# rmcar17/SpectralClusterSupertree

Hardware: AMD Instinct MI355X
Metric: top-level PCG build + Fiedler solve wall-time (s) at N taxa, 1/2/4/8 MI355X (lower is better)
Workload: dtype f64 (loop operator: fp32 image of W; fp64 renewal + confirmation)

## Files before the change

spectralclustersupertree_amd/csrc/scs_build.hip:

```cpp

#include <algorithm>

#include "scs_internal.h"

typedef unsigned long long u64;
typedef unsigned int u32;

constexpr u32 DEPTH_INF = 0xFFFFFFFFu;


__device__ __forceinline__ void rmq_offsets(int m, int a, int b, int (&o)[2]) {
    const int k = 31 - __clz(b - a);
    o[0] = k * m + a;
    o[1] = k * m + b - (1 << k);
}

template <typename K>
__device__ __forceinline__ K rmq_min(const K *__restrict__ base, int m, int a, int b) {
    int o[2];
    rmq_offsets(m, a, b, o);
    const K x = base[o[0]], y = base[o[1]];
    return x < y ? x : y;
}

// ... 659 lines not shown
        }
        if (n <= 2048) max_batch_trees = 4096;
        const int arrived = tb->late_start.empty() ? M : tb->late_start[0];
        if (wide) {
            const int rest = M - (arrived < M ? arrived : 0);
            const int k = std::max(1, (rest + 511) / 512);
            max_batch_trees = std::max(96, (rest + k - 1) / k);
        }
        if (tree_par)
            max_batch_trees = (int)std::max<size_t>(16, std::min<size_t>((size_t)max_batch_trees,
                                                                         SCS_SCRATCH_KEEP / cells_per_tree));
        if (batch_trees_env > 0) max_batch_trees = batch_trees_env;
        if (tree_par)
            max_batch_trees = (int)std::max<size_t>(1, std::min<size_t>((size_t)max_batch_trees,
                                                                        SCS_SCRATCH_KEEP / std::max<size_t>(cells_per_tree, 1)));
        size_t used = 0;
        for (int t = 0; t < M; ++t) {
            const int64_t nt = tb->h_tree_off[t + 1] - tb->h_tree_off[t];
            const int64_t m = nt - 1;
            const size_t need =
                (size_t)table_entries(m) * entry_bytes + (size_t)npad * 4 + (size_t)n_blocks * rec_bytes;
            if ((used + need > ctx->ws_limit || t - batch_start.back() >= max_batch_trees ||
                 (t == arrived && batch_start.size() == 1)) &&
                t > batch_start.back()) {
                batch_start.push_back(t);
                used = 0;
            }
            used += need;
        }
        batch_start.push_back(M);
    }
    const int n_batches = (int)batch_start.size() - 1;

    struct ev_ref {
        hipEvent_t a, b;
    } ev_total, ev_prep, ev_acc;
    for (auto &e : ctx->build_events)
        if (!e) SCS_HIP_CHECK(hipEventCreate(&e));
    ev_total = {ctx->build_events[0], ctx->build_events[1]};
    ev_prep = {ctx->build_events[2], ctx->build_events[3]};
    ev_acc = {ctx->build_events[4], ctx->build_events[5]};
    float prep_ms = 0.f, acc_ms = 0.f;
    SCS_HIP_CHECK(hipEventRecord(ev_total.a, s));

    int spec_batches = 0, spec_trees = 0;
    float spec_ms = 0.f;
    bool single_batch_spec = false;
    pooled_buf d_pos(ctx, 1), d_st(ctx, 3), d_stoff(ctx, 4), d_rec(ctx, 5), d_cells(ctx, 6);
    dev_buf d_pcol(ctx), d_lists(ctx), d_list_cnt(ctx);
    int listed_batches = 0;
    for (int bi = 0; bi < n_batches; ++bi) {
        const int t0 = batch_start[bi], t1 = batch_start[bi + 1];
        const int nb = t1 - t0;
        std::vector<int64_t> st_off(nb + 1);
        int max_levels = 0;
        int64_t max_n = 0;
        st_off[0] = 0;
        for (int t = t0; t < t1; ++t) {
            const int64_t nt = tb->h_tree_off[t + 1] - tb->h_tree_off[t];
            st_off[t - t0 + 1] = st_off[t - t0] + table_entries(nt - 1);
            max_levels = std::max(max_levels, levels_for(nt - 1));
            max_n = std::max(max_n, nt);
        }
        const size_t need_pos = (size_t)nb * npad * 4;
        const size_t need_st = (size_t)st_off[nb] * entry_bytes + 64;
        const size_t need_stoff = (size_t)(nb + 1) * 8;
        const size_t need_rec = (size_t)n_blocks * nb * rec_bytes;
        const int wide_min_trees = wide_forced ? 1 : 96;
        const bool wide_b = wide && (nb >= wide_min_trees || (groups.size() >= 8 * 256 && nb >= 16));
        if (wide_b) {
            ++spec_batches;
            spec_trees += nb;
            single_batch_spec = true;
        }
        SCS_TRY(d_pos.alloc(need_pos));
        SCS_TRY(d_st.alloc(need_st));
        SCS_TRY(d_stoff.alloc(need_stoff));
        SCS_TRY(d_rec.alloc(need_rec));

        SCS_HIP_CHECK(hipEventRecord(ev_prep.a, s));
        SCS_TRY(scs_tables_wait(ctx, tb, t1, s));
        SCS_HIP_CHECK(hipMemcpyAsync(d_stoff.p, st_off.data(), need_stoff, hipMemcpyHostToDevice, s));
        SCS_HIP_CHECK(hipMemsetAsync(d_pos.p, 0xFF, need_pos, s));
        dim3 grid_l((unsigned)((max_n + 255) / 256), (unsigned)nb);
        if (monotone) {
            k_positions_values<<<grid_l, 256, 0, s>>>(tb->d_tree_off, tb->d_leaf_taxon,
                                                      tb->d_adj_depth, tb->d_adj_val, tb->d_tree_w,
                                                      t0, (int32_t *)d_pos.p, npad,
                                                      (const int64_t *)d_stoff.p, (double *)d_st.p);
            if (max_n <= SPARSE_FUSED_MAX_LEAVES && max_levels > 1)
                k_sparse_levels_fused<double><<<(unsigned)nb, 1024, 0, s>>>(
                    tb->d_tree_off, t0, (const int64_t *)d_stoff.p, (double *)d_st.p, pick_smaller_value{});
            else
            for (int k = 1; k < max_levels; ++k)
                k_sparse_level<double><<<grid_l, 256, 0, s>>>(tb->d_tree_off, t0, k,
                                                              (const int64_t *)d_stoff.p,
                                                              (double *)d_st.p);
            if (wide_b)
                k_block_records_wide<PIPE_NG><<<dim3((unsigned)n_blocks, (unsigned)nb), 64, 0, s>>>(
                    tb->d_tree_off, t0, nb, (const int32_t *)d_pos.p, npad, (const int64_t *)d_stoff.p,
                    (const double *)d_st.p, b_row_begin, b_row_end, (unsigned char *)d_rec.p);
            else if (!scatter)
            k_block_records_mono<<<dim3((unsigned)n_blocks, (unsigned)nb), 64, 0, s>>>(
                tb->d_tree_off, t0, nb, (const int32_t *)d_pos.p, npad, (const int64_t *)d_stoff.p,
                (const double *)d_st.p, b_row_begin, b_row_end, (unsigned char *)d_rec.p);
        } else {
            k_positions_pairs<<<grid_l, 256, 0, s>>>(tb->d_tree_off, tb->d_leaf_taxon,
                                                     tb->d_adj_depth, tb->d_adj_val, tb->d_tree_w,
                                                     t0, (int32_t *)d_pos.p, npad,
                                                     (const int64_t *)d_stoff.p, (gap_entry *)d_st.p);
            if (max_n <= SPARSE_FUSED_MAX_LEAVES && max_levels > 1)
                k_sparse_levels_fused<gap_entry><<<(unsigned)nb, 1024, 0, s>>>(
                    tb->d_tree_off, t0, (const int64_t *)d_stoff.p, (gap_entry *)d_st.p, pick_shallower_pair{});
            else
            for (int k = 1; k < max_levels; ++k)
                k_sparse_level_pairs<<<grid_l, 256, 0, s>>>(tb->d_tree_off, t0, k,
                                                            (const int64_t *)d_stoff.p,
                                                            (gap_entry *)d_st.p);
            k_block_records_gen<<<dim3((unsigned)n_blocks, (unsigned)nb), 64, 0, s>>>(
                tb->d_tree_off, t0, nb, (const int32_t *)d_pos.p, npad, (const int64_t *)d_stoff.p,
                (const gap_entry *)d_st.p, b_row_begin, b_row_end, (unsigned char *)d_rec.p);
        }
        SCS_HIP_CHECK(hipEventRecord(ev_prep.b, s));

        SCS_HIP_CHECK(hipEventRecord(ev_acc.a, s));
        const unsigned nt = (unsigned)tiles.size();
        if (scatter) {
            const int64_t nbk = (max_n + 63) / 64;
            k_scatter_atomic<<<dim3((unsigned)(nbk * (nbk + 1) / 2), (unsigned)nb), 256, 0, s>>>(
                tb->d_tree_off, tb->d_leaf_taxon, t0, (const int64_t *)d_stoff.p, (const double *)d_st.p,
                g->d_w, g->ld);
        } else if (monotone) {
            mono_params mp;
            mp.tiles = (const int2 *)d_tiles.p;
            mp.rec = (const unsigned char *)d_rec.p;
            mp.pos = (const int32_t *)d_pos.p;
            mp.npad = npad;
            mp.stv = (const double *)d_st.p;
            mp.n_batch = nb;
            mp.w = w_base;
            mp.ld = g->ld;
            mp.n = n;
            mp.row_begin = b_row_begin;
            mp.row_end = b_row_end;
            mp.load_w = bi > 0;
            mp.mirror = (sym && bi == n_batches - 1) ? 1 : 0;
            mp.tile_out = shared ? (double *)d_tile_out.p : nullptr;
            mp.stamps = nullptr;
            mp.split_tiles = 0;
            mp.lists = nullptr;
            mp.list_cnt = nullptr;
            const bool stamp = scs_dbg("SCS_ACC_STAMP") && atoi(scs_dbg("SCS_ACC_STAMP"));
            if (wide_b) {
                wide_params wp;
                wp.m = mp;
                wp.groups = (const int4 *)d_groups.p;
                wp.producer_prio = 2;
                const unsigned ng = (unsigned)groups.size();
// ... 78 lines not shown
        } else {
            gen_params gp;
            gp.tiles = (const int2 *)d_tiles.p;
            gp.rec = (const unsigned char *)d_rec.p;
            gp.pos = (const int32_t *)d_pos.p;
            gp.npad = npad;
            gp.ste = (const gap_entry *)d_st.p;
            gp.n_batch = nb;
            gp.w = w_base;
            gp.ld = g->ld;
            gp.n = n;
            gp.row_begin = b_row_begin;
            gp.row_end = b_row_end;
            gp.load_w = bi > 0;
            gp.mirror = (sym && bi == n_batches - 1) ? 1 : 0;
            gp.tile_out = shared ? (double *)d_tile_out.p : nullptr;
            gp.split_tiles = 0;
            if (nt && tree_par) {
                SCS_TRY(d_cells.alloc((size_t)nb * cells_per_tree));
                gen_params ap = gp;
                ap.split_tiles = (int)nt;
                ap.load_w = 0;
                ap.mirror = 0;
                ap.tile_out = (double *)d_cells.p;
                k_accumulate_gen<true><<<nt * (unsigned)nb, MONO_TCW, 0, s>>>(ap);
                k_sum_tree_tiles<true, gen_params><<<nt * SCS_TR, MONO_TCW, 0, s>>>(gp, (const double *)d_cells.p,
                                                                                   (int)nt);
            } else if (nt) {
                if (sym) k_accumulate_gen<true><<<nt, MONO_TCW, 0, s>>>(gp);
                else k_accumulate_gen<false><<<nt, MONO_TCW, 0, s>>>(gp);
            }
        }
        SCS_HIP_CHECK(hipGetLastError());
        SCS_HIP_CHECK(hipEventRecord(ev_acc.b, s));
        if (n_batches > 1) {
            SCS_HIP_CHECK(hipEventSynchronize(ev_acc.b));
            float ms = 0.f;
            SCS_HIP_CHECK(hipEventElapsedTime(&ms, ev_prep.a, ev_prep.b));
            prep_ms += ms;
            SCS_HIP_CHECK(hipEventElapsedTime(&ms, ev_acc.a, ev_acc.b));
            acc_ms += ms;
            if (wide_b) spec_ms += ms;
        }
    }
    float exch_ms = 0.f;
    double exch_bytes = 0.0;
    if (shared && exchange_allgather) {
        ev_pair ev_x;
        SCS_TRY(ev_x.init());
        SCS_HIP_CHECK(hipEventRecord(ev_x.a, s));
        SCS_TRY(scs_comm_allgather_f64(&ctx->comm, (const double *)d_tile_out.p,
                                       (double *)d_gathered.p, chunk_doubles, s));
        k_unpack_tiles<<<(unsigned)all_tiles.size(), cols_per_tile, 0, s>>>(
            (const double *)d_gathered.p, (const int2 *)d_all_tiles.p, world,
            (int64_t)chunk_doubles, n, row_begin, row_end, g->d_w, g->ld);
        SCS_HIP_CHECK(hipGetLastError());
        SCS_HIP_CHECK(hipEventRecord(ev_x.b, s));
        SCS_HIP_CHECK(hipEventSynchronize(ev_x.b));
        SCS_HIP_CHECK(hipEventElapsedTime(&exch_ms, ev_x.a, ev_x.b));
        exch_bytes = (double)chunk_doubles * 8.0 * (world - 1);
    } else if (shared) {
        std::vector<int32_t> splits;
        SCS_TRY(scs_gather_row_splits(ctx, row_begin, row_end, n, splits));
        auto needs = [&](int dst, const int2 &t) {
            const int64_t lo = splits[dst], hi = splits[dst + 1];
            const int64_t r_lo = (int64_t)t.x * SCS_TR, r_hi = std::min<int64_t>(r_lo + SCS_TR, n);
            const int64_t c_lo = (int64_t)t.y * cols_per_tile, c_hi = std::min<int64_t>(c_lo + cols_per_tile, n);
            return (r_lo < hi && lo < r_hi) || (c_lo < hi && lo < c_hi);
        };
        std::vector<int64_t> send_off(world + 1, 0), recv_off(world + 1, 0);
        std::vector<int32_t> send_slots;
        std::vector<int2> recv_tiles;
        for (int p = 0; p < world; ++p) {
            for (size_t i = rank; i < all_tiles.size(); i += world)
                if (needs(p, all_tiles[i])) send_slots.push_back((int32_t)(i / world));
            send_off[p + 1] = (int64_t)send_slots.size() * SCS_TR * cols_per_tile;
            for (size_t i = p; i < all_tiles.size(); i += world)
                if (needs(rank, all_tiles[i])) recv_tiles.push_back(all_tiles[i]);
            recv_off[p + 1] = (int64_t)recv_tiles.size() * SCS_TR * cols_per_tile;
        }
        cached_buf d_send(ctx), d_recv(ctx);
        dev_buf d_slots(ctx), d_rtiles(ctx);
        SCS_TRY(d_send.alloc((size_t)send_off[world] * 8));
        SCS_TRY(d_recv.alloc((size_t)recv_off[world] * 8));
        SCS_TRY(d_slots.alloc(send_slots.size() * 4));
        SCS_TRY(d_rtiles.alloc(recv_tiles.size() * sizeof(int2)));
        ev_pair ev_x;
        SCS_TRY(ev_x.init());
        SCS_HIP_CHECK(hipEventRecord(ev_x.a, s));
        SCS_HIP_CHECK(hipMemcpyAsync(d_slots.p, send_slots.data(), send_slots.size() * 4,
                                     hipMemcpyHostToDevice, s));
        SCS_HIP_CHECK(hipMemcpyAsync(d_rtiles.p, recv_tiles.data(), recv_tiles.size() * sizeof(int2),
                                     hipMemcpyHostToDevice, s));
        if (!send_slots.empty())
            k_pack_tiles<<<(unsigned)send_slots.size(), 256, 0, s>>>(
                (const double *)d_tile_out.p, (const int32_t *)d_slots.p, cols_per_tile, (double *)d_send.p);
        SCS_HIP_CHECK(hipGetLastError());
        SCS_TRY(scs_comm_alltoallv_f64(&ctx->comm, (const double *)d_send.p, send_off.data(),
                                       (double *)d_recv.p, recv_off.data(), s));
        if (!recv_tiles.empty())
            k_unpack_received<<<(unsigned)recv_tiles.size(), cols_per_tile, 0, s>>>(
                (const double *)d_recv.p, (const int2 *)d_rtiles.p, n, row_begin, row_end, g->d_w,
                g->ld);
        SCS_HIP_CHECK(hipGetLastError());
        SCS_HIP_CHECK(hipEventRecord(ev_x.b, s));
        SCS_HIP_CHECK(hipEventSynchronize(ev_x.b));
        SCS_HIP_CHECK(hipEventElapsedTime(&exch_ms, ev_x.a, ev_x.b));
        exch_bytes = (double)(recv_off[world] - (recv_off[rank + 1] - recv_off[rank])) * 8.0;
    }
    SCS_HIP_CHECK(hipEventRecord(ev_total.b, s));
    SCS_HIP_CHECK(hipEventSynchronize(ev_total.b));
    SCS_TRY(scs_tables_finish(ctx, tb));
    float total_ms = 0.f;
    SCS_HIP_CHECK(hipEventElapsedTime(&total_ms, ev_total.a, ev_total.b));
    if (n_batches == 1) {
        SCS_HIP_CHECK(hipEventElapsedTime(&prep_ms, ev_prep.a, ev_prep.b));
        SCS_HIP_CHECK(hipEventElapsedTime(&acc_ms, ev_acc.a, ev_acc.b));
        if (single_batch_spec) spec_ms = acc_ms;
    }

    if (stats) {
        memset(stats, 0, sizeof(*stats));
        stats->n_taxa = n;
        stats->n_trees = M;
        stats->row_begin = row_begin;
        stats->row_end = row_end;
        stats->symmetric = shared ? 2 : (sym ? 1 : 0);
        stats->exchange_ms = exch_ms;
        stats->exchange_bytes = exch_bytes;
        stats->n_tiles = (int32_t)tiles.size();
        stats->n_batches = n_batches;
        stats->spec_batches = spec_batches;
        stats->tree_parallel_batches = tree_par ? n_batches : 0;
        stats->spec_trees = spec_trees;
        stats->listed_batches = listed_batches;
        stats->spec_ms = spec_ms;
        stats->cell_trees = (double)tiles.size() * SCS_TR * cols_per_tile * (double)M;
        stats->prep_ms = prep_ms;
        stats->accumulate_ms = acc_ms;
        stats->total_ms = total_ms;
        stats->bytes_w = 8.0 * rows * (double)n;
        stats->bytes_tables = 16.0 * (double)tb->n_leaves + 8.0 * M;
    }
    gd.g = nullptr;
    *out = g;
    return SCS_OK;
}

extern "C" int scs_graph_contract(scs_ctx *ctx, scs_graph *g, const int32_t *group_start,
                                  int32_t n_groups, scs_graph **out) {
    SCS_REQUIRE(ctx && g && group_start && out, "scs_graph_contract: null argument");
// ... 217 lines not shown
```

spectralclustersupertree_amd/csrc/scs_ctx.hip:

```cpp

#include <dlfcn.h>

#include <atomic>
#include <condition_variable>
#include <mutex>

#include "scs_internal.h"
#include "scs_arena.h"

#include <chrono>
#include <pthread.h>

#include <algorithm>
#include <cmath>

static thread_local std::string g_last_error;

void scs_set_error(const char *fmt, ...) {
    char buf[1024];
    va_list ap;
    va_start(ap, fmt);
    vsnprintf(buf, sizeof(buf), fmt, ap);
    va_end(ap);
    g_last_error = buf;
// ... 473 lines not shown

namespace {
constexpr int ARENA_DEVICES = 16;
struct device_arena {
    std::mutex mu;
    scs_arena_core core;
    std::vector<hipEvent_t> event_pool;
    std::atomic<bool> live{false};
};
device_arena g_arena[ARENA_DEVICES];

bool arena_on() {
    static const bool on = [] {
        const char *e = scs_dbg("SCS_ARENA");
        return !(e && atoi(e) == 0);
    }();
    return on;
}

void arena_init(device_arena &a) {
    if (a.live.load()) return;
    a.core.back_alloc = [](size_t bytes) -> void * {
        void *p = nullptr;
        if (driver_malloc(&p, bytes) != hipSuccess) {
            (void)hipGetLastError();
            return nullptr;
        }
        return p;
    };
    a.core.back_free = [](void *p) { driver_free(p); };
    a.core.owner_mark = [&a](const void *owner) {
        std::vector<void *> events;
        const scs_ctx *ctx = (const scs_ctx *)owner;
        for (hipStream_t s : {ctx->stream, ctx->small_stream, ctx->copy_stream}) {
            if (!s) continue;
            if (hipStreamQuery(s) == hipSuccess) continue;
            (void)hipGetLastError();
            hipEvent_t ev = nullptr;
            if (!a.event_pool.empty()) {
                ev = a.event_pool.back();
                a.event_pool.pop_back();
            } else if (hipEventCreateWithFlags(&ev, hipEventDisableTiming) != hipSuccess) {
                (void)hipGetLastError();
                hipStreamSynchronize(s);
                continue;
            }
            hipEventRecord(ev, s);
            events.push_back((void *)ev);
        }
        return events;
    };
    a.core.event_done = [](void *e) {
        if (hipEventQuery((hipEvent_t)e) == hipSuccess) return true;
        (void)hipGetLastError();
        return false;
    };
    a.core.event_wait = [](void *e) { hipEventSynchronize((hipEvent_t)e); };
    a.core.event_recycle = [&a](void *e) { a.event_pool.push_back((hipEvent_t)e); };
    a.live.store(true);
}
}

hipError_t scs_dev_malloc_impl(scs_ctx *ctx, void **p, size_t bytes) {
    if (!ctx || !arena_on() || ctx->device < 0 || ctx->device >= ARENA_DEVICES) return driver_malloc(p, bytes);
    device_arena &a = g_arena[ctx->device];
    std::lock_guard<std::mutex> lock(a.mu);
    arena_init(a);
// ... 106 lines not shown
        if (b.p == p) b.in_use = false;
        if (!b.in_use) free_bytes += b.bytes;
    }
    while (free_bytes > SCS_PINNED_KEEP) {
        size_t pick = ctx->pinned.size();
        for (size_t i = 0; i < ctx->pinned.size(); ++i)
            if (!ctx->pinned[i].in_use && (pick == ctx->pinned.size() || ctx->pinned[i].bytes > ctx->pinned[pick].bytes))
                pick = i;
        if (pick == ctx->pinned.size()) break;
        free_bytes -= ctx->pinned[pick].bytes;
        hipHostFree(ctx->pinned[pick].p);
        ctx->pinned.erase(ctx->pinned.begin() + pick);
    }
}

void scs_block_drop_free(scs_ctx *ctx) {
    (void)ctx;
}

void scs_block_release(scs_ctx *ctx, void *p) {
    (void)ctx;
    if (p) scs_dev_free(p);
}

extern "C" int scs_ctx_destroy(scs_ctx *ctx) {
    if (!ctx) return SCS_OK;
    hipSetDevice(ctx->device);
    if (ctx->stream) {
        hipStreamSynchronize(ctx->stream);
    }
    scs_comm_destroy(&ctx->comm);
    if (ctx->copy_stream) hipStreamSynchronize(ctx->copy_stream);
    if (ctx->small_stream) hipStreamSynchronize(ctx->small_stream);
    if (ctx->h_report) hipHostFree(ctx->h_report);
    for (auto &sl : ctx->scratch)
        if (sl.p) scs_dev_free(sl.p);
    for (auto &e : ctx->build_events)
        if (e) hipEventDestroy(e);
    for (auto &e : ctx->solve_events)
        if (e) hipEventDestroy(e);
    if (ctx->w_cache) scs_dev_free(ctx->w_cache);
    if (ctx->w32_cache) scs_dev_free(ctx->w32_cache);
    for (auto &b : ctx->pinned)
        if (!b.in_use) hipHostFree(b.p);
    for (auto e : ctx->event_pool) hipEventDestroy(e);
    for (auto &sl : ctx->small_slots) {
        if (sl.done) hipEventDestroy(sl.done);
        if (sl.dev) scs_dev_free(sl.dev);
        if (sl.host) hipHostFree(sl.host);
        if (sl.scratch) scs_dev_free(sl.scratch);
    }
    ctx->small_slots.clear();
    if (ctx->h_flags) hipHostFree(ctx->h_flags);
    arena_ctx_gone(ctx);
    if (ctx->copy_stream) hipStreamDestroy(ctx->copy_stream);
    if (ctx->small_stream) hipStreamDestroy(ctx->small_stream);
    if (ctx->stream) hipStreamDestroy(ctx->stream);
    delete ctx;
    return SCS_OK;
}

extern "C" int scs_ctx_trim(scs_ctx *ctx, int64_t keep_bytes) {
    SCS_REQUIRE(ctx != nullptr, "scs_ctx_trim: null context");
    SCS_HIP_CHECK(hipSetDevice(ctx->device));
    SCS_HIP_CHECK(hipStreamSynchronize(ctx->stream));
    if (ctx->small_stream) SCS_HIP_CHECK(hipStreamSynchronize(ctx->small_stream));
    std::lock_guard<std::mutex> lock(ctx->cache_mu);
    if (ctx->w_cache) {
        scs_dev_free(ctx->w_cache);
        ctx->w_cache = nullptr;
        ctx->w_cache_bytes = 0;
    }
    if (ctx->w32_cache) {
        scs_dev_free(ctx->w32_cache);
        ctx->w32_cache = nullptr;
        ctx->w32_cache_bytes = 0;
    }
    const size_t keep = keep_bytes > 0 ? (size_t)keep_bytes : 0;
    if (keep == 0) {
        for (auto &sl : ctx->scratch) {
            if (sl.p) scs_dev_free(sl.p);
            sl.p = nullptr;
            sl.cap = 0;
        }
        for (auto &sl : ctx->small_slots) {
            if (sl.busy) continue;
            if (sl.dev) scs_dev_free(sl.dev);
            if (sl.host) hipHostFree(sl.host);
            if (sl.scratch) scs_dev_free(sl.scratch);
            sl.dev = nullptr;
            sl.host = nullptr;
            sl.cap = 0;
            sl.scratch = nullptr;
            sl.scratch_cap = 0;
        }
    }
    arena_trim(ctx->device, keep);
    for (size_t i = 0; i < ctx->pinned.size();) {
        if (!ctx->pinned[i].in_use && keep == 0) {
// ... 25 lines not shown

__global__ __launch_bounds__(256) void k_validate_tables(const int32_t *__restrict__ leaf_taxon,
                                                          const int32_t *__restrict__ adj_depth,
                                                          int64_t n_leaves, int32_t n_taxa,
                                                          unsigned *__restrict__ flags) {
    unsigned bad = 0;
    for (int64_t p = (int64_t)blockIdx.x * blockDim.x + threadIdx.x; p < n_leaves;
         p += (int64_t)gridDim.x * blockDim.x) {
        const int32_t tx = leaf_taxon[p];
        if (tx < 0 || tx >= n_taxa) bad |= 1u;
        if (adj_depth[p] < 0) bad |= 2u;
    }
    if (bad) atomicOr(flags, bad);
}

extern "C" int scs_host_alloc(size_t bytes, void **out) {
    SCS_REQUIRE(out != nullptr, "scs_host_alloc: null output");
    void *p = nullptr;
    hipError_t e = hipHostMalloc(&p, bytes ? bytes : 1, hipHostMallocDefault);
    if (e != hipSuccess) {
        (void)hipGetLastError();
        scs_set_error("scs_host_alloc: cannot pin %zu bytes: %s", bytes, hipGetErrorString(e));
        return SCS_ENOMEM;
    }
    *out = p;
    return SCS_OK;
}

extern "C" int scs_host_free(void *p) {
    if (p) SCS_HIP_CHECK(hipHostFree(p));
    return SCS_OK;
}

int scs_tables_wait(scs_ctx *ctx, const scs_tables *t, int32_t t_end, hipStream_t stream) {
    for (size_t c = 0; c < t->late_ev.size(); ++c)
        if (t->late_start[c] < t_end) SCS_HIP_CHECK(hipStreamWaitEvent(stream, t->late_ev[c], 0));
    return SCS_OK;
}

int scs_tables_finish(scs_ctx *ctx, const scs_tables *t) {
    if (t->late_ev.empty()) return SCS_OK;
    hipError_t e = hipSuccess;
    for (hipEvent_t ev : t->late_ev) {
        const hipError_t w = hipEventSynchronize(ev);
        if (e == hipSuccess) e = w;
        hipEventDestroy(ev);
    }
    t->late_ev.clear();
    t->late_start.clear();
    if (e == hipSuccess && ctx->copy_stream) e = hipStreamSynchronize(ctx->copy_stream);
    unsigned bad = 0;
    if (e == hipSuccess) e = hipMemcpy(&bad, t->d_flags, 4, hipMemcpyDeviceToHost);
    if (e != hipSuccess) {
        scs_set_error("table upload failed: %s", hipGetErrorString(e));
        return SCS_EHIP;
    }
    if (bad) {
        scs_set_error("scs_tables_upload: %s", (bad & 1u) ? "a leaf_taxon entry is out of range [0, n_taxa)"
                                                          : "an adj_depth entry is negative");
        return SCS_EINVAL;
    }
    return SCS_OK;
}

static bool scs_is_pinned(const void *p) {
    hipPointerAttribute_t a;
    if (hipPointerGetAttributes(&a, p) != hipSuccess) {
        (void)hipGetLastError();
        return false;
// ... 197 lines not shown
    auto up256 = [](size_t b) { return (b + 255) / 256 * 256; };
    const size_t o_off = 0;
    const size_t o_tax = o_off + up256(((size_t)n_trees + 1) * 8);
    const size_t o_dep = o_tax + up256((size_t)L * 4);
    const size_t o_val = o_dep + up256((size_t)L * 4);
    const size_t o_w = o_val + up256((size_t)L * 8);
    const size_t o_flag = o_w + up256((size_t)n_trees * 8);
    void *block = nullptr;
    SCS_TRY(scs_block_alloc(ctx, o_flag + 256, &block));
    auto *t = new scs_tables();
    t->n_taxa = n_taxa;
    t->n_trees = n_trees;
    t->n_leaves = L;
    t->max_leaves = (int32_t)max_leaves;
    t->h_tree_off.assign(tree_off, tree_off + n_trees + 1);
    t->d_block = block;
    char *base = (char *)block;
    t->d_tree_off = (int64_t *)(base + o_off);
    t->d_leaf_taxon = (int32_t *)(base + o_tax);
    t->d_adj_depth = (int32_t *)(base + o_dep);
    t->d_adj_val = (double *)(base + o_val);
    t->d_tree_w = (double *)(base + o_w);
    unsigned *d_flags = (unsigned *)(base + o_flag);
    t->d_flags = d_flags;
    hipStream_t s = ctx->stream;
    int32_t first = n_trees, chunk = n_trees;
    if (n_taxa > 2048 && (size_t)L * 16 >= ((size_t)8 << 20) && scs_is_pinned(leaf_taxon) &&
        scs_is_pinned(adj_depth) && scs_is_pinned(adj_val)) {
        const double avg = std::max((double)L / n_trees - 1.0, 1.0);
        const double table_bytes = (std::floor(std::log2(avg)) + 1.0) * avg * 8.0;
        const int32_t per = (int32_t)std::min(256.0, std::max(64.0, 600e6 / table_bytes));
        if (n_trees >= 2 * per || n_trees - per >= 32) {
            first = std::min(per, 64);
            chunk = per;
        }
    }
    const int64_t L0 = tree_off[first];
    hipError_t e = hipMemsetAsync(d_flags, 0, 4, s);
    if (e == hipSuccess) e = hipMemcpyAsync(t->d_tree_off, tree_off, ((size_t)n_trees + 1) * 8, hipMemcpyHostToDevice, s);
    if (e == hipSuccess && L0) e = hipMemcpyAsync(t->d_leaf_taxon, leaf_taxon, (size_t)L0 * 4, hipMemcpyHostToDevice, s);
    if (e == hipSuccess && L0) e = hipMemcpyAsync(t->d_adj_depth, adj_depth, (size_t)L0 * 4, hipMemcpyHostToDevice, s);
    if (e == hipSuccess && L0) e = hipMemcpyAsync(t->d_adj_val, adj_val, (size_t)L0 * 8, hipMemcpyHostToDevice, s);
    if (e == hipSuccess) e = hipMemcpyAsync(t->d_tree_w, tree_w, (size_t)n_trees * 8, hipMemcpyHostToDevice, s);
    if (e == hipSuccess) {
        const int grid = (int)std::min<int64_t>((L0 + 255) / 256 + 1, 4096);
        k_validate_tables<<<grid, 256, 0, s>>>(t->d_leaf_taxon, t->d_adj_depth, L0, n_taxa, d_flags);
        e = hipGetLastError();
    }
    if (e == hipSuccess) e = hipMemcpyAsync(ctx->h_flags, d_flags, 4, hipMemcpyDeviceToHost, s);
    if (e == hipSuccess) e = hipStreamSynchronize(s);
    if (e == hipSuccess && first < n_trees) {
        if (!ctx->copy_stream) e = hipStreamCreateWithFlags(&ctx->copy_stream, hipStreamNonBlocking);
        hipStream_t cs = ctx->copy_stream;
        for (int32_t a = first; a < n_trees && e == hipSuccess; a += chunk) {
            const int32_t b = std::min(n_trees, a + chunk);
            const int64_t p0 = tree_off[a], cnt = tree_off[b] - tree_off[a];
            e = hipMemcpyAsync(t->d_leaf_taxon + p0, leaf_taxon + p0, (size_t)cnt * 4, hipMemcpyHostToDevice, cs);
            if (e == hipSuccess) e = hipMemcpyAsync(t->d_adj_depth + p0, adj_depth + p0, (size_t)cnt * 4, hipMemcpyHostToDevice, cs);
            if (e == hipSuccess) e = hipMemcpyAsync(t->d_adj_val + p0, adj_val + p0, (size_t)cnt * 8, hipMemcpyHostToDevice, cs);
            hipEvent_t ev = nullptr;
            if (e == hipSuccess) e = hipEventCreateWithFlags(&ev, hipEventDisableTiming);
            if (e == hipSuccess) e = hipEventRecord(ev, cs);
            if (e == hipSuccess) {
                t->late_start.push_back(a);
                t->late_ev.push_back(ev);
            } else if (ev) {
                hipEventDestroy(ev);
            }
            if (e == hipSuccess) {
                const int grid = (int)std::min<int64_t>((cnt + 255) / 256 + 1, 4096);
                k_validate_tables<<<grid, 256, 0, cs>>>(t->d_leaf_taxon + p0, t->d_adj_depth + p0, cnt, n_taxa, d_flags);
                e = hipGetLastError();
            }
        }
    }
    if (e != hipSuccess) {
        scs_tables_free(ctx, t);
        scs_set_error("table upload failed: %s", hipGetErrorString(e));
        return e == hipErrorOutOfMemory ? SCS_ENOMEM : SCS_EHIP;
    }
    const unsigned bad = *ctx->h_flags;
    if (bad) {
        scs_tables_free(ctx, t);
        scs_set_error("scs_tables_upload: %s", (bad & 1u) ? "a leaf_taxon entry is out of range [0, n_taxa)"
                                                          : "an adj_depth entry is negative");
        return SCS_EINVAL;
    }
    *out = t;
    return SCS_OK;
}
```

spectralclustersupertree_amd/csrc/scs_internal.h:

```cpp
#pragma once

#include <hip/hip_runtime.h>

#include <cstdarg>
#include <cstdint>
#include <cstdio>
#include <cstring>
#include <mutex>
#include <string>
#include <vector>

#include "../../include/scs_hip.h"

void scs_set_error(const char *fmt, ...);

#define SCS_HIP_CHECK(expr)                                                                  \
    do {                                                                                     \
        hipError_t e_ = (expr);                                                              \
        if (e_ != hipSuccess) {                                                              \
            scs_set_error("%s failed: %s (%s:%d)", #expr, hipGetErrorString(e_), __FILE__,   \
                          __LINE__);                                                         \
            return (e_ == hipErrorOutOfMemory) ? SCS_ENOMEM : SCS_EHIP;                      \
        }                                                                                    \
    } while (0)
// ... 36 lines not shown
constexpr int SCS_LD_ALIGN = 512;

constexpr size_t SCS_SCRATCH_KEEP = (size_t)1 << 30;
constexpr size_t SCS_PINNED_KEEP = (size_t)2 << 30;

struct scs_ctx;
int scs_block_alloc(scs_ctx *ctx, size_t bytes, void **out);
void scs_block_release(scs_ctx *ctx, void *p);
void scs_block_drop_free(scs_ctx *ctx);
int scs_pinned_get(scs_ctx *ctx, size_t bytes, void **out);
void scs_pinned_release(scs_ctx *ctx, void *p);

struct scs_local_group;

struct scs_comm {
    int rank = 0;
    int world = 1;
    int kind = 0;
    void *rccl_comm = nullptr;
    scs_local_group *group = nullptr;
};

int scs_comm_allgather_f64(scs_comm *comm, const double *sendbuf, double *recvbuf, size_t count,
                           hipStream_t stream);
int scs_comm_alltoallv_f64(scs_comm *comm, const double *sendbuf, const int64_t *send_off,
                           double *recvbuf, const int64_t *recv_off, hipStream_t stream);
int scs_comm_init_rccl(scs_comm *comm, int rank, int world, const void *uid);
int scs_comm_destroy(scs_comm *comm);

struct scs_ctx {
    int device = 0;
    hipStream_t stream = nullptr;
    hipStream_t copy_stream = nullptr;
    scs_comm comm;
    int n_cu = 256;
    int max_lds_bytes = 65536;
    size_t ws_limit = 0;
    double *h_report = nullptr;
    double *d_report = nullptr;
    unsigned long long report_seq = 0;
    struct scratch_slot {
        void *p = nullptr;
        size_t cap = 0;
    } scratch[8];
    hipEvent_t build_events[6] = {nullptr, nullptr, nullptr, nullptr, nullptr, nullptr};
    hipEvent_t solve_events[2] = {nullptr, nullptr};
    double *w_cache = nullptr;
    size_t w_cache_bytes = 0;
    float *w32_cache = nullptr;
    size_t w32_cache_bytes = 0;
    struct cached_block {
        void *p;
        size_t bytes;
        bool in_use;
    };
    std::mutex cache_mu;
    std::vector<cached_block> blocks;
    std::vector<cached_block> pinned;
    std::vector<hipEvent_t> event_pool;
    unsigned *h_flags = nullptr;
    struct small_slot {
        unsigned char *host = nullptr;
        unsigned char *dev = nullptr;
        size_t cap = 0;
        hipEvent_t done = nullptr;
        bool busy = false;
        size_t o_maps = 0, maps_bytes = 0, o_lam = 0, lam_bytes = 0, o_w = 0, w_bytes = 0;
        unsigned char *scratch = nullptr;
        size_t scratch_cap = 0;
    };
    std::vector<small_slot> small_slots;
    hipStream_t small_stream = nullptr;
};

struct scs_tables {
    int32_t n_taxa = 0;
    int32_t n_trees = 0;
    int64_t n_leaves = 0;
    int32_t max_leaves = 0;
    std::vector<int64_t> h_tree_off;
    void *d_block = nullptr;
    int64_t *d_tree_off = nullptr;
    int32_t *d_leaf_taxon = nullptr;
    int32_t *d_adj_depth = nullptr;
    double *d_adj_val = nullptr;
    double *d_tree_w = nullptr;
    mutable std::vector<int32_t> late_start;
    mutable std::vector<hipEvent_t> late_ev;
    unsigned *d_flags = nullptr;
};

int scs_tables_wait(scs_ctx *ctx, const scs_tables *t, int32_t t_end, hipStream_t stream);
int scs_tables_finish(scs_ctx *ctx, const scs_tables *t);

struct mf_data {
    const scs_tables *tb = nullptr;
    int64_t *d_stack_off = nullptr;
    int64_t stack_total = 0;
    int b_cap = 0;
    int chunks = 1;
    double *st_val = nullptr, *st_sum = nullptr;
    int32_t *st_dep = nullptr;
    double *sm_val = nullptr, *sm_sum = nullptr, *cy_pa = nullptr, *cy_ps = nullptr;
    int32_t *sm_dep = nullptr, *cy_dep = nullptr, *sm_cnt = nullptr, *sm_root = nullptr, *cy_cnt = nullptr;
    double *x = nullptr;
    double *y = nullptr;
    double *slabs = nullptr;
    int slabs_b = 0;
    int64_t n_apply = 0;
};

struct scs_graph {
    mf_data *mf = nullptr;
    int32_t n = 0;
    int32_t row_begin = 0;
    int32_t row_end = 0;
    int64_t ld = 0;
    double *d_w = nullptr;
    int32_t col0 = 0;
    bool upper = false;
    size_t w_bytes = 0;
    bool w_block = false;
    bool have_deg = false;
    void *deg_stage = nullptr;
    float *d_w32 = nullptr;
// ... 57 lines not shown
```

Before: 0.01432.

## Pipeline per-batch table prep on a high-priority stream with double-buffered scratch

Per-batch preparation (positions, sparse tables, block records) moves to a separate high-priority stream and uses two alternating scratch buffer sets, so the next batch's prep can overlap the current batch's accumulation. The per-batch host synchronisation that existed only for timing is removed, and timings are now read from per-batch events at the end. Prep inside a batch is also split at late-arriving table chunk boundaries, so each piece waits only on the chunks it needs. Upload chunks are capped in size and validation runs once after upload. The cost is extra memory for the second buffer set and more events and cross-stream dependencies. The new path only applies when there is more than one batch.

Result: faster. 0.01404 (median of 6 runs) (-2.0%).

```diff
diff --git a/spectralclustersupertree_amd/csrc/scs_build.hip b/spectralclustersupertree_amd/csrc/scs_build.hip
--- a/spectralclustersupertree_amd/csrc/scs_build.hip
+++ b/spectralclustersupertree_amd/csrc/scs_build.hip
@@ -715,98 +715,144 @@
     }
     const int n_batches = (int)batch_start.size() - 1;
 
-    struct ev_ref {
-        hipEvent_t a, b;
-    } ev_total, ev_prep, ev_acc;
+    const bool piped = n_batches > 1;
+    hipStream_t ps = s;
+    if (piped) {
+        if (!ctx->prep_stream) {
+            int least = 0, greatest = 0;
+            SCS_HIP_CHECK(hipDeviceGetStreamPriorityRange(&least, &greatest));
+            SCS_HIP_CHECK(hipStreamCreateWithPriority(&ctx->prep_stream, hipStreamNonBlocking, greatest));
+        }
+        ps = ctx->prep_stream;
+    }
+
     for (auto &e : ctx->build_events)
         if (!e) SCS_HIP_CHECK(hipEventCreate(&e));
-    ev_total = {ctx->build_events[0], ctx->build_events[1]};
-    ev_prep = {ctx->build_events[2], ctx->build_events[3]};
-    ev_acc = {ctx->build_events[4], ctx->build_events[5]};
+    hipEvent_t ev_total_a = ctx->build_events[0], ev_total_b = ctx->build_events[1];
+    while (piped && ctx->batch_events.size() < (size_t)n_batches * 4) {
+        hipEvent_t e = nullptr;
+        SCS_HIP_CHECK(hipEventCreate(&e));
+        ctx->batch_events.push_back(e);
+    }
+    auto bev = [&](int bi, int k) { return piped ? ctx->batch_events[(size_t)bi * 4 + k] : ctx->build_events[2 + k]; };
     float prep_ms = 0.f, acc_ms = 0.f;
-    SCS_HIP_CHECK(hipEventRecord(ev_total.a, s));
+    SCS_HIP_CHECK(hipEventRecord(ev_total_a, s));
+    if (piped) SCS_HIP_CHECK(hipStreamWaitEvent(ps, ev_total_a, 0));
+
+    std::vector<std::vector<int64_t>> st_offs((size_t)n_batches);
+    std::vector<int> b_levels((size_t)n_batches);
+    std::vector<int64_t> b_max_n((size_t)n_batches);
+    size_t need_max[2][4] = {{0, 0, 0, 0}, {0, 0, 0, 0}};
+    for (int bi = 0; bi < n_batches; ++bi) {
+        const int t0 = batch_start[bi], t1 = batch_start[bi + 1];
+        const int nb = t1 - t0;
+        std::vector<int64_t> &st_off = st_offs[(size_t)bi];
+        st_off.assign((size_t)nb + 1, 0);
+        int max_levels = 0;
+        int64_t max_n = 0;
+        for (int t = t0; t < t1; ++t) {
+            const int64_t nt = tb->h_tree_off[t + 1] - tb->h_tree_off[t];
+            st_off[t - t0 + 1] = st_off[t - t0] + table_entries(nt - 1);
+            max_levels = std::max(max_levels, levels_for(nt - 1));
+            max_n = std::max(max_n, nt);
+        }
+        b_levels[(size_t)bi] = max_levels;
+        b_max_n[(size_t)bi] = max_n;
+        size_t *nm = need_max[bi & 1];
+        nm[0] = std::max(nm[0], (size_t)nb * npad * 4);
+        nm[1] = std::max(nm[1], (size_t)st_off[nb] * entry_bytes + 64);
+        nm[2] = std::max(nm[2], (size_t)(nb + 1) * 8);
+        nm[3] = std::max(nm[3], (size_t)n_blocks * nb * rec_bytes);
+    }
+    pooled_buf d_pos_s[2] = {pooled_buf(ctx, 1), pooled_buf(ctx, 7)};
+    pooled_buf d_st_s[2] = {pooled_buf(ctx, 3), pooled_buf(ctx, 8)};
+    pooled_buf d_stoff_s[2] = {pooled_buf(ctx, 4), pooled_buf(ctx, 9)};
+    pooled_buf d_rec_s[2] = {pooled_buf(ctx, 5), pooled_buf(ctx, 10)};
+    for (int k = 0; k < (n_batches > 1 ? 2 : 1); ++k) {
+        SCS_TRY(d_pos_s[k].alloc(need_max[k][0]));
+        SCS_TRY(d_st_s[k].alloc(need_max[k][1]));
+        SCS_TRY(d_stoff_s[k].alloc(need_max[k][2]));
+        SCS_TRY(d_rec_s[k].alloc(need_max[k][3]));
+    }
 
     int spec_batches = 0, spec_trees = 0;
     float spec_ms = 0.f;
-    bool single_batch_spec = false;
-    pooled_buf d_pos(ctx, 1), d_st(ctx, 3), d_stoff(ctx, 4), d_rec(ctx, 5), d_cells(ctx, 6);
+    std::vector<char> b_wide((size_t)n_batches, 0);
+    pooled_buf d_cells(ctx, 6);
     dev_buf d_pcol(ctx), d_lists(ctx), d_list_cnt(ctx);
     int listed_batches = 0;
     for (int bi = 0; bi < n_batches; ++bi) {
         const int t0 = batch_start[bi], t1 = batch_start[bi + 1];
         const int nb = t1 - t0;
-        std::vector<int64_t> st_off(nb + 1);
-        int max_levels = 0;
-        int64_t max_n = 0;
-        st_off[0] = 0;
-        for (int t = t0; t < t1; ++t) {
-            const int64_t nt = tb->h_tree_off[t + 1] - tb->h_tree_off[t];
-            st_off[t - t0 + 1] = st_off[t - t0] + table_entries(nt - 1);
-            max_levels = std::max(max_levels, levels_for(nt - 1));
-            max_n = std::max(max_n, nt);
-        }
+        const std::vector<int64_t> &st_off = st_offs[(size_t)bi];
+        const int max_levels = b_levels[(size_t)bi];
+        const int64_t max_n = b_max_n[(size_t)bi];
+        pooled_buf &d_pos = d_pos_s[bi & 1], &d_st = d_st_s[bi & 1], &d_stoff = d_stoff_s[bi & 1],
+                   &d_rec = d_rec_s[bi & 1];
         const size_t need_pos = (size_t)nb * npad * 4;
-        const size_t need_st = (size_t)st_off[nb] * entry_bytes + 64;
         const size_t need_stoff = (size_t)(nb + 1) * 8;
-        const size_t need_rec = (size_t)n_blocks * nb * rec_bytes;
         const int wide_min_trees = wide_forced ? 1 : 96;
         const bool wide_b = wide && (nb >= wide_min_trees || (groups.size() >= 8 * 256 && nb >= 16));
         if (wide_b) {
             ++spec_batches;
             spec_trees += nb;
-            single_batch_spec = true;
-        }
-        SCS_TRY(d_pos.alloc(need_pos));
-        SCS_TRY(d_st.alloc(need_st));
-        SCS_TRY(d_stoff.alloc(need_stoff));
-        SCS_TRY(d_rec.alloc(need_rec));
-
-        SCS_HIP_CHECK(hipEventRecord(ev_prep.a, s));
-        SCS_TRY(scs_tables_wait(ctx, tb, t1, s));
-        SCS_HIP_CHECK(hipMemcpyAsync(d_stoff.p, st_off.data(), need_stoff, hipMemcpyHostToDevice, s));
-        SCS_HIP_CHECK(hipMemsetAsync(d_pos.p, 0xFF, need_pos, s));
-        dim3 grid_l((unsigned)((max_n + 255) / 256), (unsigned)nb);
-        if (monotone) {
-            k_positions_values<<<grid_l, 256, 0, s>>>(tb->d_tree_off, tb->d_leaf_taxon,
-                                                      tb->d_adj_depth, tb->d_adj_val, tb->d_tree_w,
-                                                      t0, (int32_t *)d_pos.p, npad,
-                                                      (const int64_t *)d_stoff.p, (double *)d_st.p);
-            if (max_n <= SPARSE_FUSED_MAX_LEAVES && max_levels > 1)
-                k_sparse_levels_fused<double><<<(unsigned)nb, 1024, 0, s>>>(
-                    tb->d_tree_off, t0, (const int64_t *)d_stoff.p, (double *)d_st.p, pick_smaller_value{});
-            else
-            for (int k = 1; k < max_levels; ++k)
-                k_sparse_level<double><<<grid_l, 256, 0, s>>>(tb->d_tree_off, t0, k,
-                                                              (const int64_t *)d_stoff.p,
-                                                              (double *)d_st.p);
-            if (wide_b)
-                k_block_records_wide<PIPE_NG><<<dim3((unsigned)n_blocks, (unsigned)nb), 64, 0, s>>>(
-                    tb->d_tree_off, t0, nb, (const int32_t *)d_pos.p, npad, (const int64_t *)d_stoff.p,
-                    (const double *)d_st.p, b_row_begin, b_row_end, (unsigned char *)d_rec.p);
-            else if (!scatter)
-            k_block_records_mono<<<dim3((unsigned)n_blocks, (unsigned)nb), 64, 0, s>>>(
-                tb->d_tree_off, t0, nb, (const int32_t *)d_pos.p, npad, (const int64_t *)d_stoff.p,
-                (const double *)d_st.p, b_row_begin, b_row_end, (unsigned char *)d_rec.p);
-        } else {
-            k_positions_pairs<<<grid_l, 256, 0, s>>>(tb->d_tree_off, tb->d_leaf_taxon,
-                                                     tb->d_adj_depth, tb->d_adj_val, tb->d_tree_w,
-                                                     t0, (int32_t *)d_pos.p, npad,
-                                                     (const int64_t *)d_stoff.p, (gap_entry *)d_st.p);
-            if (max_n <= SPARSE_FUSED_MAX_LEAVES && max_levels > 1)
-                k_sparse_levels_fused<gap_entry><<<(unsigned)nb, 1024, 0, s>>>(
-                    tb->d_tree_off, t0, (const int64_t *)d_stoff.p, (gap_entry *)d_st.p, pick_shallower_pair{});
-            else
-            for (int k = 1; k < max_levels; ++k)
-                k_sparse_level_pairs<<<grid_l, 256, 0, s>>>(tb->d_tree_off, t0, k,
-                                                            (const int64_t *)d_stoff.p,
-                                                            (gap_entry *)d_st.p);
-            k_block_records_gen<<<dim3((unsigned)n_blocks, (unsigned)nb), 64, 0, s>>>(
-                tb->d_tree_off, t0, nb, (const int32_t *)d_pos.p, npad, (const int64_t *)d_stoff.p,
-                (const gap_entry *)d_st.p, b_row_begin, b_row_end, (unsigned char *)d_rec.p);
-        }
-        SCS_HIP_CHECK(hipEventRecord(ev_prep.b, s));
-
-        SCS_HIP_CHECK(hipEventRecord(ev_acc.a, s));
+            b_wide[(size_t)bi] = 1;
+        }
+
+        SCS_HIP_CHECK(hipEventRecord(bev(bi, 0), s));
+        if (piped && bi >= 2) SCS_HIP_CHECK(hipStreamWaitEvent(ps, bev(bi - 1, 3), 0));
+        SCS_HIP_CHECK(hipMemcpyAsync(d_stoff.p, st_off.data(), need_stoff, hipMemcpyHostToDevice, ps));
+        SCS_HIP_CHECK(hipMemsetAsync(d_pos.p, 0xFF, need_pos, ps));
+        std::vector<int> cuts{t0};
+        for (int32_t ls : tb->late_start)
+            if (ls > t0 && ls < t1) cuts.push_back(ls);
+        cuts.push_back(t1);
+        for (size_t ci = 0; ci + 1 < cuts.size(); ++ci) {
+            const int a = cuts[ci], o = a - t0, cnt = cuts[ci + 1] - a;
+            SCS_TRY(scs_tables_wait(ctx, tb, a, a + cnt, ps));
+            int32_t *pos_a = (int32_t *)d_pos.p + (int64_t)o * npad;
+            const int64_t *stoff_a = (const int64_t *)d_stoff.p + o;
+            unsigned char *rec_a = (unsigned char *)d_rec.p + (size_t)o * rec_bytes;
+            dim3 grid_l((unsigned)((max_n + 255) / 256), (unsigned)cnt);
+            if (monotone) {
+                k_positions_values<<<grid_l, 256, 0, ps>>>(tb->d_tree_off, tb->d_leaf_taxon, tb->d_adj_depth,
+                                                           tb->d_adj_val, tb->d_tree_w, a, pos_a, npad, stoff_a,
+                                                           (double *)d_st.p);
+                if (max_n <= SPARSE_FUSED_MAX_LEAVES && max_levels > 1)
+                    k_sparse_levels_fused<double><<<(unsigned)cnt, 1024, 0, ps>>>(
+                        tb->d_tree_off, a, stoff_a, (double *)d_st.p, pick_smaller_value{});
+                else
+                    for (int k = 1; k < max_levels; ++k)
+                        k_sparse_level<double><<<grid_l, 256, 0, ps>>>(tb->d_tree_off, a, k, stoff_a,
+                                                                       (double *)d_st.p);
+                if (wide_b)
+                    k_block_records_wide<PIPE_NG><<<dim3((unsigned)n_blocks, (unsigned)cnt), 64, 0, ps>>>(
+                        tb->d_tree_off, a, nb, pos_a, npad, stoff_a, (const double *)d_st.p, b_row_begin,
+                        b_row_end, rec_a);
+                else if (!scatter)
+                    k_block_records_mono<<<dim3((unsigned)n_blocks, (unsigned)cnt), 64, 0, ps>>>(
+                        tb->d_tree_off, a, nb, pos_a, npad, stoff_a, (const double *)d_st.p, b_row_begin,
+                        b_row_end, rec_a);
+            } else {
+                k_positions_pairs<<<grid_l, 256, 0, ps>>>(tb->d_tree_off, tb->d_leaf_taxon, tb->d_adj_depth,
+                                                          tb->d_adj_val, tb->d_tree_w, a, pos_a, npad, stoff_a,
+                                                          (gap_entry *)d_st.p);
+                if (max_n <= SPARSE_FUSED_MAX_LEAVES && max_levels > 1)
+                    k_sparse_levels_fused<gap_entry><<<(unsigned)cnt, 1024, 0, ps>>>(
+                        tb->d_tree_off, a, stoff_a, (gap_entry *)d_st.p, pick_shallower_pair{});
+                else
+                    for (int k = 1; k < max_levels; ++k)
+                        k_sparse_level_pairs<<<grid_l, 256, 0, ps>>>(tb->d_tree_off, a, k, stoff_a,
+                                                                     (gap_entry *)d_st.p);
+                k_block_records_gen<<<dim3((unsigned)n_blocks, (unsigned)cnt), 64, 0, ps>>>(
+                    tb->d_tree_off, a, nb, pos_a, npad, stoff_a, (const gap_entry *)d_st.p, b_row_begin,
+                    b_row_end, rec_a);
+            }
+        }
+        SCS_HIP_CHECK(hipGetLastError());
+        SCS_HIP_CHECK(hipEventRecord(bev(bi, 1), ps));
+        if (piped) SCS_HIP_CHECK(hipStreamWaitEvent(s, bev(bi, 1), 0));
+        SCS_HIP_CHECK(hipEventRecord(bev(bi, 2), s));
         const unsigned nt = (unsigned)tiles.size();
         if (scatter) {
             const int64_t nbk = (max_n + 63) / 64;
@@ -951,16 +997,7 @@
             }
         }
         SCS_HIP_CHECK(hipGetLastError());
-        SCS_HIP_CHECK(hipEventRecord(ev_acc.b, s));
-        if (n_batches > 1) {
-            SCS_HIP_CHECK(hipEventSynchronize(ev_acc.b));
-            float ms = 0.f;
-            SCS_HIP_CHECK(hipEventElapsedTime(&ms, ev_prep.a, ev_prep.b));
-            prep_ms += ms;
-            SCS_HIP_CHECK(hipEventElapsedTime(&ms, ev_acc.a, ev_acc.b));
-            acc_ms += ms;
-            if (wide_b) spec_ms += ms;
-        }
+        SCS_HIP_CHECK(hipEventRecord(bev(bi, 3), s));
     }
     float exch_ms = 0.f;
     double exch_bytes = 0.0;
@@ -1027,15 +1064,18 @@
         SCS_HIP_CHECK(hipEventElapsedTime(&exch_ms, ev_x.a, ev_x.b));
         exch_bytes = (double)(recv_off[world] - (recv_off[rank + 1] - recv_off[rank])) * 8.0;
     }
-    SCS_HIP_CHECK(hipEventRecord(ev_total.b, s));
-    SCS_HIP_CHECK(hipEventSynchronize(ev_total.b));
+    SCS_HIP_CHECK(hipEventRecord(ev_total_b, s));
+    SCS_HIP_CHECK(hipEventSynchronize(ev_total_b));
     SCS_TRY(scs_tables_finish(ctx, tb));
     float total_ms = 0.f;
-    SCS_HIP_CHECK(hipEventElapsedTime(&total_ms, ev_total.a, ev_total.b));
-    if (n_batches == 1) {
-        SCS_HIP_CHECK(hipEventElapsedTime(&prep_ms, ev_prep.a, ev_prep.b));
-        SCS_HIP_CHECK(hipEventElapsedTime(&acc_ms, ev_acc.a, ev_acc.b));
-        if (single_batch_spec) spec_ms = acc_ms;
+    SCS_HIP_CHECK(hipEventElapsedTime(&total_ms, ev_total_a, ev_total_b));
+    for (int bi = 0; bi < n_batches; ++bi) {
+        float ms = 0.f;
+        SCS_HIP_CHECK(hipEventElapsedTime(&ms, bev(bi, 0), bev(bi, 2)));
+        prep_ms += ms;
+        SCS_HIP_CHECK(hipEventElapsedTime(&ms, bev(bi, 2), bev(bi, 3)));
+        acc_ms += ms;
+        if (b_wide[(size_t)bi]) spec_ms += ms;
     }
 
     if (stats) {
diff --git a/spectralclustersupertree_amd/csrc/scs_ctx.hip b/spectralclustersupertree_amd/csrc/scs_ctx.hip
--- a/spectralclustersupertree_amd/csrc/scs_ctx.hip
+++ b/spectralclustersupertree_amd/csrc/scs_ctx.hip
@@ -529,7 +529,7 @@
     a.core.owner_mark = [&a](const void *owner) {
         std::vector<void *> events;
         const scs_ctx *ctx = (const scs_ctx *)owner;
-        for (hipStream_t s : {ctx->stream, ctx->small_stream, ctx->copy_stream}) {
+        for (hipStream_t s : {ctx->stream, ctx->small_stream, ctx->copy_stream, ctx->prep_stream}) {
             if (!s) continue;
             if (hipStreamQuery(s) == hipSuccess) continue;
             (void)hipGetLastError();
@@ -702,11 +702,13 @@
     scs_comm_destroy(&ctx->comm);
     if (ctx->copy_stream) hipStreamSynchronize(ctx->copy_stream);
     if (ctx->small_stream) hipStreamSynchronize(ctx->small_stream);
+    if (ctx->prep_stream) hipStreamSynchronize(ctx->prep_stream);
     if (ctx->h_report) hipHostFree(ctx->h_report);
     for (auto &sl : ctx->scratch)
         if (sl.p) scs_dev_free(sl.p);
     for (auto &e : ctx->build_events)
         if (e) hipEventDestroy(e);
+    for (auto e : ctx->batch_events) hipEventDestroy(e);
     for (auto &e : ctx->solve_events)
         if (e) hipEventDestroy(e);
     if (ctx->w_cache) scs_dev_free(ctx->w_cache);
@@ -725,6 +727,7 @@
     arena_ctx_gone(ctx);
     if (ctx->copy_stream) hipStreamDestroy(ctx->copy_stream);
     if (ctx->small_stream) hipStreamDestroy(ctx->small_stream);
+    if (ctx->prep_stream) hipStreamDestroy(ctx->prep_stream);
     if (ctx->stream) hipStreamDestroy(ctx->stream);
     delete ctx;
     return SCS_OK;
@@ -735,6 +738,7 @@
     SCS_HIP_CHECK(hipSetDevice(ctx->device));
     SCS_HIP_CHECK(hipStreamSynchronize(ctx->stream));
     if (ctx->small_stream) SCS_HIP_CHECK(hipStreamSynchronize(ctx->small_stream));
+    if (ctx->prep_stream) SCS_HIP_CHECK(hipStreamSynchronize(ctx->prep_stream));
     std::lock_guard<std::mutex> lock(ctx->cache_mu);
     if (ctx->w_cache) {
         scs_dev_free(ctx->w_cache);
@@ -826,9 +830,12 @@
     return SCS_OK;
 }
 
-int scs_tables_wait(scs_ctx *ctx, const scs_tables *t, int32_t t_end, hipStream_t stream) {
-    for (size_t c = 0; c < t->late_ev.size(); ++c)
-        if (t->late_start[c] < t_end) SCS_HIP_CHECK(hipStreamWaitEvent(stream, t->late_ev[c], 0));
+int scs_tables_wait(scs_ctx *ctx, const scs_tables *t, int32_t t_begin, int32_t t_end, hipStream_t stream) {
+    for (size_t c = 0; c < t->late_ev.size(); ++c) {
+        const int32_t c_end = c + 1 < t->late_start.size() ? t->late_start[c + 1] : t->n_trees;
+        if (t->late_start[c] < t_end && c_end > t_begin)
+            SCS_HIP_CHECK(hipStreamWaitEvent(stream, t->late_ev[c], 0));
+    }
     return SCS_OK;
 }
 
@@ -1092,7 +1099,7 @@
         const int32_t per = (int32_t)std::min(256.0, std::max(64.0, 600e6 / table_bytes));
         if (n_trees >= 2 * per || n_trees - per >= 32) {
             first = std::min(per, 64);
-            chunk = per;
+            chunk = std::min(per, 128);
         }
     }
     const int64_t L0 = tree_off[first];
@@ -1127,11 +1134,12 @@
             } else if (ev) {
                 hipEventDestroy(ev);
             }
-            if (e == hipSuccess) {
-                const int grid = (int)std::min<int64_t>((cnt + 255) / 256 + 1, 4096);
-                k_validate_tables<<<grid, 256, 0, cs>>>(t->d_leaf_taxon + p0, t->d_adj_depth + p0, cnt, n_taxa, d_flags);
-                e = hipGetLastError();
-            }
+        }
+        if (e == hipSuccess) {
+            const int64_t p0 = tree_off[first], cnt = L - p0;
+            const int grid = (int)std::min<int64_t>((cnt + 255) / 256 + 1, 4096);
+            k_validate_tables<<<grid, 256, 0, cs>>>(t->d_leaf_taxon + p0, t->d_adj_depth + p0, cnt, n_taxa, d_flags);
+            e = hipGetLastError();
         }
     }
     if (e != hipSuccess) {
diff --git a/spectralclustersupertree_amd/csrc/scs_internal.h b/spectralclustersupertree_amd/csrc/scs_internal.h
--- a/spectralclustersupertree_amd/csrc/scs_internal.h
+++ b/spectralclustersupertree_amd/csrc/scs_internal.h
@@ -92,6 +92,7 @@
     int device = 0;
     hipStream_t stream = nullptr;
     hipStream_t copy_stream = nullptr;
+    hipStream_t prep_stream = nullptr;
     scs_comm comm;
     int n_cu = 256;
     int max_lds_bytes = 65536;
@@ -102,8 +103,9 @@
     struct scratch_slot {
         void *p = nullptr;
         size_t cap = 0;
-    } scratch[8];
+    } scratch[12];
     hipEvent_t build_events[6] = {nullptr, nullptr, nullptr, nullptr, nullptr, nullptr};
+    std::vector<hipEvent_t> batch_events;
     hipEvent_t solve_events[2] = {nullptr, nullptr};
     double *w_cache = nullptr;
     size_t w_cache_bytes = 0;
@@ -150,7 +152,7 @@
     unsigned *d_flags = nullptr;
 };
 
-int scs_tables_wait(scs_ctx *ctx, const scs_tables *t, int32_t t_end, hipStream_t stream);
+int scs_tables_wait(scs_ctx *ctx, const scs_tables *t, int32_t t_begin, int32_t t_end, hipStream_t stream);
 int scs_tables_finish(scs_ctx *ctx, const scs_tables *t);
 
 struct mf_data {
```
